# jyjblrd/Low-Cost-Mocap

Hardware: AMD Instinct MI355X
Metric: triangulated 3D markers/sec at 8 cams x 16 markers (higher is better)
Workload: dtype f64

## Files before the change

### low-cost-mocap_amd/csrc/frame_bb.hip

```cpp
#include "mocap_device.hpp"
#include "kernels.hpp"
#include <cstdlib>
#include "frame_common.hpp"
#include "bb_fold.hpp"

namespace mocap {

constexpr int kBBThreads = 256;
constexpr int kBBWaves = kBBThreads / 64;
constexpr int kBBRecs = kBBThreads + 64;
constexpr int bb_cw(int C) { return C <= 8 ? 1 : 2; }
constexpr uint32_t bb_rec_bytes(int CW) { return 24u + 8u * (uint32_t)CW; }
constexpr bool bb_group_rows(int CT, int ML, int RL) { return CT > 0 && ML > 0 && RL > 0 && CT * ML < 0xFF && (ML & (ML - 1)) == 0; }

constexpr int bb_wg_per_cu(int RL) { return RL == 48 ? 5 : 4; }
constexpr size_t kBBCacheEntry = 4;
constexpr int kBBLdsSlack = 1024;
struct BBLayout {
  size_t bxy, bxy_nx, cnt_nx, bt, rbound, seedkey, slot_key, claimw, recs, rpk, scr, scr_bytes, goff, gcnt, outslot, boff, bnb, seedgh, slot_g, cnt,
      misc, bpl, nh, hits, act, root_blob, root_cam, nact, bnl, bv, pkbase, seen, bcache, total;
  int ncache;
  __host__ __device__ static size_t al(size_t x, size_t a) { return (x + a - 1) / a * a; }
  __host__ __device__ BBLayout(int C, int M, int R, int CW, int wg_per_cu, bool row_words = false) {
    size_t o = 0;
    auto take = [&](size_t bytes, size_t a) {
      o = al(o, a);
      const size_t at = o;
      o += bytes;
      return at;
    };
    bxy = take(sizeof(float2) * (size_t)C * M, 16);
    bxy_nx = take(sizeof(float2) * (size_t)C * M, 16);
    cnt_nx = take(4 * (size_t)C, 4);
    bt = take(sizeof(double) * 10 * ((size_t)C * M + 1), 16);
    rbound = take(8 * (size_t)R, 8);
    claimw = take(8 * (size_t)C, 8);
    pkbase = take(8 * (size_t)CW * R, 8);
    scr = seedkey = take(8 * (size_t)R, 8);
    slot_key = take(8 * (size_t)kBBWaves * R, 8);
    recs = take(8 * (size_t)kBBRecs, 8);
    rpk = take(8 * (size_t)kBBRecs * CW, 8);
    seedgh = take(4 * (size_t)R, 4);
    slot_g = take(4 * (size_t)kBBWaves * R, 4);
    scr_bytes = o - scr;
    goff = take(4 * (size_t)(R + 1), 4);
    gcnt = take(4 * (size_t)R, 4);
    outslot = take(4 * (size_t)R, 4);
    boff = take(4 * (size_t)(R + 1), 4);
    bnb = take(4 * (size_t)R, 4);
    cnt = take(4 * (size_t)C, 4);
    misc = take(4 * 16, 4);
    bpl = take(2 * (size_t)R, 2);
    seen = take(2 * (size_t)R, 2);
    nh = take((size_t)R * C, row_words ? 8 : 1);
    hits = take((size_t)R * C * M, 1);
    act = take((size_t)R * C, row_words ? 8 : 1);
    root_blob = take((size_t)R, 1);
    root_cam = take((size_t)R, 1);
    nact = take((size_t)R, 1);
    bnl = take((size_t)R, 1);
    bv = take((size_t)R, 1);
    bcache = take(0, 4);
    ncache = 0;
    const size_t per_entry = kBBCacheEntry;
    for (int per_cu = wg_per_cu; per_cu >= 1; per_cu--) {
      const size_t lim = ((size_t)160 * 1024 / per_cu - kBBLdsSlack) / 256 * 256;
      if (lim >= o + per_entry * 64) {
        const size_t n = (lim - o) / per_entry;
        ncache = (int)(n > 1024 ? 1024 : n);
        break;
      }
    }
    o += per_entry * (size_t)ncache;
    total = al(o, 16);
  }
};

static int bb_fixed_slots(int C, int M, int R) {
  const char* e = getenv("MOCAP_BB_FIXED_LAYOUT");
  if (e && e[0] == '0') return 0;
  if (C == 8 && M == 16 && R <= 48) return 48;
  if (C == 8 && M == 16 && R <= 64) return 64;
  return 0;
}
static int frame_bb_root_slots(int C, int M, int R) {
  const int f = bb_fixed_slots(C, M, R);
  return f ? f : R;
}
size_t frame_bb_lds_bytes(int C, int M, int R) { return BBLayout(C, M, frame_bb_root_slots(C, M, R), bb_cw(C), bb_wg_per_cu(bb_fixed_slots(C, M, R)), bb_fixed_slots(C, M, R) != 0).total; }
static size_t frame_bb_lds_bytes_min(int C, int M, int R) {
  const BBLayout L(C, M, frame_bb_root_slots(C, M, R), bb_cw(C), bb_wg_per_cu(bb_fixed_slots(C, M, R)), bb_fixed_slots(C, M, R) != 0);
  return L.total - kBBCacheEntry * (size_t)L.ncache;
}
bool frame_bb_fits(int C, int M, int R) {
  return C >= 2 && C <= 16 && M >= 1 && M <= 64 && R >= 1 && R <= 255 && frame_bb_lds_bytes_min(C, M, R) <= (size_t)128 * 1024;
}

template <int CW, uint32_t NONE = 0xFFu>
struct Packed {
  unsigned long long w[CW];
  __device__ __forceinline__ void clear() {
#pragma unroll
    for (int k = 0; k < CW; k++) w[k] = NONE * 0x0101010101010101ull;
  }
  __device__ __forceinline__ void set(int c, uint32_t idx) {
    if (CW == 1)
      w[0] ^= (unsigned long long)(idx ^ NONE) << (8 * c);
    else
      w[c >> 3] ^= (unsigned long long)(idx ^ NONE) << (8 * (c & 7));
  }
  __device__ __forceinline__ uint32_t get(int c) const {
    return CW == 1 ? (uint32_t)(w[0] >> (8 * c)) & 0xFFu : (uint32_t)(w[c >> 3] >> (8 * (c & 7))) & 0xFFu;
  }
};

template <int CT, bool PERK = false>
struct BBCamTables {
  const double* base;
  static constexpr int C = CT;
  static constexpr int kPq = PERK ? 12 * CT * CT : 12 * CT;
  __device__ __forceinline__ ctab_t pq(size_t off) const { return as_ctab(base + off); }
  __device__ __forceinline__ ctab_t rt(size_t off) const { return as_ctab(base + kPq + off); }
  __device__ __forceinline__ ctab_t k4(size_t off) const { return as_ctab(base + kPq + 12 * CT + off); }
  __device__ __forceinline__ const double* f() const { return base + kPq + 16 * CT; }
};
template <bool PERK>
struct BBCamTables<0, PERK> {
  const double* base;
  int C;
  __device__ __forceinline__ ctab_t pq(size_t off) const { return as_ctab(base + off); }
  __device__ __forceinline__ ctab_t rt(size_t off) const { return as_ctab(base + (PERK ? 12 * C * C : 12 * C) + off); }
  __device__ __forceinline__ ctab_t k4(size_t off) const { return as_ctab(base + (PERK ? 12 * C * C + 12 * C : 24 * C) + off); }
  __device__ __forceinline__ const double* f() const { return base + (PERK ? 12 * C * C + 16 * C : 28 * C); }
};

enum { kPrioEval = 0, kPrioSeed = 1, kPrioPhase = 2, kPrioSerial = 3 };
template <int P>
__device__ __forceinline__ void bb_prio() {
  __builtin_amdgcn_s_setprio(P);
}

template <bool F32R, int CW, int CT, int ML, int RL, bool PERK = false>
struct BBState {
  static constexpr int T = kBBThreads, W = kBBWaves;
  static constexpr bool ROWS = bb_group_rows(CT, ML, RL);
  static constexpr uint32_t kNone = ROWS ? (uint32_t)(CT * ML) : 0xFFu;
  typedef Packed<CW, kNone> Pk;
  static_assert(!ROWS || (CT == 8 && CW == 1), "a row of nh / act as one word: eight cameras");
  __device__ __forceinline__ unsigned long long row_word64(const uint8_t* rows, int r) const { return ((const unsigned long long*)rows)[r]; }
  __device__ static __forceinline__ uint32_t byte_of(unsigned long long w, uint32_t k) { return (uint32_t)(w >> (8u * k)) & 0xFFu; }
  static constexpr bool PLIST = CT > 0 && ML > 0 && RL > 0 && ML < 32 && CT * ML <= 256 && (ML & (ML - 1)) == 0;
  __device__ __forceinline__ uint32_t gbyte(int c, uint32_t k) const { return ROWS ? (uint32_t)c * (uint32_t)ML + k : k; }
  __device__ __forceinline__ size_t grow(int c, uint32_t b) const { return ROWS ? (size_t)b : (size_t)c * M + b; }
  const FrameArgs& p;
  BBCamTables<CT, PERK> cv;
  const int C_, M, R, RS;
  int tid, lane, wave;
  __device__ __forceinline__ void fresh_tid() {
    int t = tid;
    asm volatile("" : "+v"(t));
    tid = t;
    lane = t & 63;
    wave = t >> 6;
  }
  __device__ __forceinline__ int cn() const { return CT > 0 ? CT : C_; }
  enum { PC_OTHER = 0, PC_PAIRS0, PC_PAIRS1, PC_B1_TABLE, PC_ROW_COPY, PC_PHASE_C, PC_SEED_PASS, PC_SEED_PUSH, PC_EVAL, PC_TEST, PC_PHASE_E, PC_COUNT };
#ifdef MOCAP_BB_PHASE_CLOCKS
  uint32_t pc_last = 0, pc_sum[PC_COUNT] = {};
  template <int PH>
  __device__ __forceinline__ void pc_mark() {
    if (__builtin_amdgcn_readfirstlane((int)threadIdx.x >> 6) == 0) {
      const uint32_t now = (uint32_t)__builtin_readcyclecounter();
      pc_sum[PH] += now - pc_last;
      pc_last = now;
    }
  }
  __device__ __forceinline__ void pc_start() { pc_last = (uint32_t)__builtin_readcyclecounter(); }
  __device__ __forceinline__ void pc_flush() const {
    if (threadIdx.x == 0 && !p.n_frames_dev)
      for (int k = 0; k < PC_COUNT; k++) atomicAdd(&p.status[p.n_frames + k], (int)(pc_sum[k] >> 8));
  }
#else
  template <int PH>
  __device__ __forceinline__ void pc_mark() {}
  __device__ __forceinline__ void pc_start() {}
  __device__ __forceinline__ void pc_flush() const {}
#endif
  double* bt;
  float2 *bxy, *bxy_nx;
  int32_t* cnt_nx;
  unsigned long long *rbound, *seedkey, *slot_key, *claimw, *rpk;
  struct BRec { uint32_t gh, rs; };
  BRec* recs;
  uint32_t *goff, *gcnt, *boff, *bnb, *seedgh, *slot_g;
  int32_t *outslot, *cnt, *misc;
  uint16_t* bpl;
  uint8_t *nh, *hits, *act, *root_blob, *root_cam, *nact, *bnl, *bv;
  float* bcache;
  unsigned long long* pkbase;
  uint16_t* seen;
  int ncache;
  unsigned char* scr;
  size_t scr_bytes;
  static constexpr unsigned long long kInfBits = 0x7ff0000000000000ull;

  __device__ BBState(const FrameArgs& p_, unsigned char* smem)
      : p(p_), C_(p_.cv.C), M(ML > 0 ? ML : p_.M), R(p_.K_max), RS(RL > 0 ? RL : p_.K_max), tid(threadIdx.x), lane(threadIdx.x & 63), wave(threadIdx.x >> 6) {
    const int C = cn();
    {
      const unsigned long long ta = (unsigned long long)(uintptr_t)p_.cv.Pq;
      uint32_t tlo = (uint32_t)__builtin_amdgcn_readfirstlane((int)(uint32_t)ta);
      uint32_t thi = (uint32_t)__builtin_amdgcn_readfirstlane((int)(uint32_t)(ta >> 32));
      asm volatile("" : "+s"(tlo), "+s"(thi));
      cv.base = (const double*)(uintptr_t)(((unsigned long long)thi << 32) | tlo);
      if constexpr (CT == 0) cv.C = C;
    }
    const BBLayout L(C, M, RS, CW, bb_wg_per_cu(RL), ROWS);
    bt = (double*)(smem + L.bt);
    bxy = (float2*)(smem + L.bxy);
    bxy_nx = (float2*)(smem + L.bxy_nx);
    cnt_nx = (int32_t*)(smem + L.cnt_nx);
    rbound = (unsigned long long*)(smem + L.rbound);
    seedkey = (unsigned long long*)(smem + L.seedkey);
    slot_key = (unsigned long long*)(smem + L.slot_key);
    claimw = (unsigned long long*)(smem + L.claimw);
    recs = (BRec*)(smem + L.recs);
    rpk = (unsigned long long*)(smem + L.rpk);
    goff = (uint32_t*)(smem + L.goff);
    gcnt = (uint32_t*)(smem + L.gcnt);
    outslot = (int32_t*)(smem + L.outslot);
    boff = (uint32_t*)(smem + L.boff);
    bnb = (uint32_t*)(smem + L.bnb);
    seedgh = (uint32_t*)(smem + L.seedgh);
    slot_g = (uint32_t*)(smem + L.slot_g);
    cnt = (int32_t*)(smem + L.cnt);
    misc = (int32_t*)(smem + L.misc);
    bpl = (uint16_t*)(smem + L.bpl);
    nh = (uint8_t*)(smem + L.nh);
    hits = (uint8_t*)(smem + L.hits);
    act = (uint8_t*)(smem + L.act);
    root_blob = (uint8_t*)(smem + L.root_blob);
    root_cam = (uint8_t*)(smem + L.root_cam);
    nact = (uint8_t*)(smem + L.nact);
    bnl = (uint8_t*)(smem + L.bnl);
    bv = (uint8_t*)(smem + L.bv);
    scr = smem + L.scr;
    scr_bytes = L.scr_bytes;
    bcache = (float*)(smem + L.bcache);
    pkbase = (unsigned long long*)(smem + L.pkbase);
    seen = (uint16_t*)(smem + L.seen);
    ncache = L.ncache;
  }

  struct Line { double a, b, c, den, rden; };
  __device__ __forceinline__ Line epiline(int r, int i) const { return epiline_of(root_cam[r], root_blob[r], i); }
  __device__ __forceinline__ Line epiline_of(int rc, int rb, int i) const {
    const int C = cn();
    const double* Fm = cv.f() + 9 * ((size_t)rc * C + i);
    const float2 rp = bxy[(size_t)rc * M + rb];
    const double x = (double)rp.x, y = (double)rp.y;
    double a = Fm[0] * x + Fm[1] * y + Fm[2];
    double b = Fm[3] * x + Fm[4] * y + Fm[5];
    double c = Fm[6] * x + Fm[7] * y + Fm[8];
    double nu = a * a + b * b;
    nu = nu != 0.0 ? 1.0 / sqrt(nu) : 1.0;
    a *= nu;
    b *= nu;
    c *= nu;
    if (F32R) {
      a = (double)(float)a;
      b = (double)(float)b;
      c = (double)(float)c;
    }
    Line L;
    L.a = a;
    L.b = b;
    L.c = c;
    L.den = sqrt(a * a + b * b);
    L.rden = recip_refined(L.den);
    return L;
  }

  template <bool CHAIN>
  __device__ __forceinline__ unsigned long long match_pairs(const Line& mine, int pair_r, int pair_i, int n_pairs, int gs_shift,
                                                            int cam = 0, int Mi_chain = 0) {
    const int C = cn();
    const int GS = 1 << gs_shift, PPS = 64 >> gs_shift;
    const int k = lane & (GS - 1), q = lane >> gs_shift;
    const int gl0 = lane & ~(GS - 1);
    const unsigned long long gall = gs_shift == 6 ? ~0ull : ((1ull << GS) - 1ull);
    unsigned long long claims = 0ull;
    for (int s0 = 0; s0 < n_pairs; s0 += PPS) {
      const int src = s0 + q;
      const bool has = src < n_pairs;
      const int sl = has ? src : 0;
      const double la = __shfl(mine.a, sl), lb = __shfl(mine.b, sl), lc = __shfl(mine.c, sl);
      const double lden = __shfl(mine.den, sl), lrden = __shfl(mine.rden, sl);
      const int r = __shfl(pair_r, sl);
      const int i = CHAIN ? cam : __shfl(pair_i, sl);
      const int Mi = has ? (CHAIN ? Mi_chain : cnt[i]) : 0;
      const bool valid = k < Mi;
      float2 pt = make_float2(0.f, 0.f);
      double d = 0.0;
      bool hit = false;
      if (valid) {
        pt = bxy[(size_t)i * M + k];
        const double num = fabs(la * (double)pt.x + lb * (double)pt.y + lc);
        d = div_by(num, lden, lrden);
        hit = d < p.gate_px;
      }
      const unsigned long long wm = __ballot(hit);
      const unsigned long long gm = (wm >> gl0) & gall;
      int rank = 0;
      const unsigned int dlo = (unsigned int)__double_as_longlong(d), dhi = (unsigned int)(__double_as_longlong(d) >> 32);
      for (unsigned long long mm = wm; mm;) {
        const int j = __ffsll((long long)mm) - 1;
        mm &= mm - 1;
        const double dj = __longlong_as_double(((long long)__builtin_amdgcn_readlane((int)dhi, j) << 32) |
                                               (unsigned int)__builtin_amdgcn_readlane((int)dlo, j));
        const bool mine_grp = (j & ~(GS - 1)) == gl0 && j != lane;
        rank += (hit && mine_grp && (dj < d || (dj == d && j < lane))) ? 1 : 0;
      }
      if (hit) hits[((size_t)r * C + i) * M + rank] = (uint8_t)gbyte(i, (uint32_t)k);
      const unsigned long long g0 = (__ballot(hit && rank == 0) >> gl0) & gall;
      bool same = false;
      if (valid && g0) {
        const float2 p0 = bxy[(size_t)i * M + (__ffsll((long long)g0) - 1)];
        same = pt.x == p0.x && pt.y == p0.y;
      }
      const unsigned long long cw = __ballot(same);
      if (CHAIN) {
        for (int sh = 0; sh < 64; sh += GS) claims |= (cw >> sh) & gall;
      }
      if (has && k == 0) {
        nh[(size_t)r * C + i] = (uint8_t)__popcll(gm);
        if (!CHAIN) {
          const unsigned long long cm = (cw >> gl0) & gall;
          if (cm) atomicOr(&claimw[i], cm);
        }
      }
    }
    return claims;
  }

  __device__ __forceinline__ void prefetch_lds(int64_t frame) const {
    const int C = cn();
    const float* src = p.blobs + (size_t)frame * C * M * 2;
    const int n_dw = C * M * 2;
    for (int base = wave * 64; base < n_dw; base += T)
      if (base + lane < n_dw)
        __builtin_amdgcn_global_load_lds((const __attribute__((address_space(1))) void*)(src + base + lane),
                                         (__attribute__((address_space(3))) void*)((float*)bxy_nx + base), 4, 0, 0);
    if (wave == 0 && lane < C)
      __builtin_amdgcn_global_load_lds((const __attribute__((address_space(1))) void*)(p.counts + (size_t)frame * C + lane),
                                       (__attribute__((address_space(3))) void*)cnt_nx, 4, 0, 0);
  }
  __device__ __forceinline__ void stage(int64_t frame) {
    fresh_tid();
    const int C = cn();
    float2* t = bxy;
    bxy = bxy_nx;
    bxy_nx = t;
    if (tid < C) {
      const int n = cnt_nx[tid];
      cnt[tid] = n < 0 ? 0 : (n > M ? M : n);
      claimw[tid] = 0ull;
    }
    if (tid == 0) {
      misc[MI_STATUS] = 0;
      misc[MI_OMAX] = 0;
    }
  }

  __device__ void match() {
    fresh_tid();
    const int C = cn();
    __syncthreads();
    int gs_shift = 0;
    while ((1 << gs_shift) < M) gs_shift++;
    const int n0 = cnt[0] < R ? cnt[0] : R;
    {
      for (int r = tid; r < n0; r += T) {
        root_cam[r] = 0;
        root_blob[r] = (uint8_t)r;
      }
      if (tid == 0 && cnt[0] > R) misc[MI_STATUS] |= MOCAP_ST_ROOT_OVERFLOW_;
    }
    __syncthreads();
    auto U_of = [&](int j) {
      const int n = cnt[j];
      return ~claimw[j] & (n >= 64 ? ~0ull : ((1ull << n) - 1ull));
    };
    int n_prov = 0, n_ppairs = 0;
    bool pre = false;
    uint8_t* nh_s = nullptr;
    uint8_t* hits_s = nullptr;
    unsigned long long* pclaim = (unsigned long long*)scr;
    uint8_t* plist = act;
    uint32_t* p_end = goff;
    {
      int Mmax = 0;
      for (int c = 1; c < C; c++) Mmax = cnt[c] > Mmax ? cnt[c] : Mmax;
#pragma nounroll
      for (int stage_ = 0; stage_ < 2; stage_++) {
        const int stage = __builtin_amdgcn_readfirstlane(stage_);
        int NP = n0 * (C - 1);
        if (stage == 1) {
          block_sync_lds();
          pc_mark<PC_PAIRS0>();
          if constexpr (PLIST) {
#pragma unroll
            for (int j = 1; j < CT; j++) {
              const uint32_t U = ~((const uint32_t*)claimw)[2 * j] & ((1u << cnt[j]) - 1u);
              if (lane < ML && ((U >> lane) & 1u)) plist[__builtin_amdgcn_mbcnt_lo(U, (uint32_t)n_prov)] = (uint8_t)(j * ML + lane);
              n_prov += __popc(U);
              n_ppairs += __popc(U) * (CT - 1 - j);
              if (lane == 0) p_end[j] = ((uint32_t)n_ppairs << 16) | (uint32_t)n_prov;
            }
            wave_lds_sync();
          } else
          for (int j = 1; j < C; j++) {
            const int np = __popcll(U_of(j));
            n_prov += np;
            n_ppairs += np * (C - 1 - j);
          }
          pre = n_prov <= 64 && (size_t)n_prov * C * (8 + 1 + (size_t)M) <= scr_bytes;
          if (!pre) break;
          nh_s = (uint8_t*)(pclaim + (size_t)n_prov * C);
          hits_s = nh_s + (size_t)n_prov * C;
          NP = n_ppairs;
        }
        for (int base = wave * 64; base < NP; base += W * 64) {
          const int pi = base + lane;
          const bool have = pi < NP;
          int r = 0, i = 1, Mi = 0;
          Line L = {0, 0, 0, 1, 1};
          if (have) {
            if (stage == 0) {
              r = pi / (C - 1);
              i = 1 + (pi - r * (C - 1));
              L = epiline(r, i);
            } else if constexpr (PLIST) {
              int j = 1;
              uint32_t before = 0;
              const uint32_t key = ((uint32_t)pi << 16) | 0xFFFFu;
              uint32_t pe[CT > 2 ? CT - 2 : 1];
#pragma unroll
              for (int jj = 1; jj <= CT - 2; jj++) pe[jj - 1] = p_end[jj];
#pragma unroll
              for (int jj = 1; jj <= CT - 2; jj++) {
                const bool ge = key >= pe[jj - 1];
                j += ge ? 1 : 0;
                before = ge ? pe[jj - 1] : before;
              }
              const uint32_t acc = before >> 16, pb = before & 0xFFFFu;
              uint32_t ord, off;
              divmod_tiny((uint32_t)pi - acc, (uint32_t)(CT - 1 - j), ord, off);
              r = (int)(pb + ord);
              const int k = plist[r] & (ML - 1);
              i = j + 1 + (int)off;
              L = epiline_of(j, k, i);
            } else {
              int j = 1, acc = 0, pb = 0, span = C - 2;
              unsigned long long U = 0ull;
              for (; j <= C - 2; j++) {
                span = C - 1 - j;
                U = U_of(j);
                const int nj = __popcll(U) * span;
                if (pi < acc + nj) break;
                acc += nj;
                pb += __popcll(U);
              }
              uint32_t ord, off;
              divmod_tiny((uint32_t)(pi - acc), (uint32_t)span, ord, off);
              for (uint32_t t = 0; t < ord; t++) U &= U - 1;
              const int k = __ffsll((long long)U) - 1;
              i = j + 1 + (int)off;
              r = pb + (int)ord;
              L = epiline_of(j, k, i);
            }
            Mi = cnt[i];
          }
          const float2* pts = bxy + (size_t)i * M;
          auto dist = [&](int k) {
            const float2 pt = pts[k];
            return div_by(fabs(L.a * (double)pt.x + L.b * (double)pt.y + L.c), L.den, L.rden);
          };
          unsigned long long hm = 0ull;
          double bd0 = __builtin_huge_val();
          int bk0 = 0;
          if constexpr (ROWS) {
#pragma unroll 4
            for (int k = 0; k < Mmax; k++)
              if (k < Mi) {
                const double d = dist(k);
                if (d < p.gate_px) {
                  hm |= 1ull << k;
                  if (d < bd0) {
                    bd0 = d;
                    bk0 = k;
                  }
                }
              }
          } else
#pragma unroll 4
          for (int k = 0; k < Mmax; k++)
            if (k < Mi && dist(k) < p.gate_px) hm |= 1ull << k;
          uint8_t* nhp = stage == 0 ? nh : nh_s;
          uint8_t* hl = (stage == 0 ? hits : hits_s) + ((size_t)r * C + i) * M;
          if (have) nhp[(size_t)r * C + i] = (uint8_t)__popcll(hm);
          unsigned long long rem = hm, claim = 0ull;
          int pos = 0;
          float2 p0 = make_float2(0.f, 0.f);
          if constexpr (ROWS) {
            if (hm) {
              hl[0] = (uint8_t)gbyte(i, (uint32_t)bk0);
              claim = hm;
              if (hm & (hm - 1ull)) {
                claim = 0ull;
                p0 = pts[bk0];
                for (unsigned long long t = hm; t; t &= t - 1) {
                  const int k = __ffsll((long long)t) - 1;
                  const float2 q = pts[k];
                  if (q.x == p0.x && q.y == p0.y) claim |= 1ull << k;
                }
              }
              rem = hm & ~(1ull << bk0);
              pos = 1;
            }
          }
          while (__ballot(rem != 0ull)) {
            if (rem) {
              double bd = __builtin_huge_val();
              int bk = 0;
              if (ROWS && !(rem & (rem - 1ull))) {
                bk = __ffsll((long long)rem) - 1;
              } else
              for (unsigned long long t = rem; t; t &= t - 1) {
                const int k = __ffsll((long long)t) - 1;
                const double d = dist(k);
                if (d < bd) {
                  bd = d;
                  bk = k;
                }
              }
              hl[pos] = (uint8_t)gbyte(i, (uint32_t)bk);
              if (!ROWS && pos == 0) {
                p0 = pts[bk];
                for (unsigned long long t = hm; t; t &= t - 1) {
                  const int k = __ffsll((long long)t) - 1;
                  const float2 q = pts[k];
                  if (q.x == p0.x && q.y == p0.y) claim |= 1ull << k;
                }
              }
              rem &= ~(1ull << bk);
              pos++;
            }
          }
          if (stage == 0) {
            if (claim) atomicOr(&claimw[i], claim);
          } else if (have) {
            pclaim[(size_t)r * C + i] = claim;
          }
        }
      }
    }
    const int NL = M * ((C - 1) * (C - 2) / 2);
    const bool spec = F32R && (size_t)NL * 20 + 8 <= scr_bytes;
    double* sp_den = (double*)scr;
    float* sp_abc = (float*)(sp_den + NL);
    auto sp_base = [&](int j) { return M * ((j - 1) * (C - 1) - (j - 1) * j / 2); };
    if (spec && !pre) {
      int tot = 0;
      for (int j = 1; j <= C - 2; j++) {
        const int n = cnt[j];
        const unsigned long long U = ~claimw[j] & (n >= 64 ? ~0ull : ((1ull << n) - 1ull));
        tot += __popcll(U) * (C - 1 - j);
      }
      for (int l = tid; l < tot; l += T) {
        int j = 1, acc = 0, span = C - 2;
        unsigned long long U = 0ull;
        for (; j <= C - 2; j++) {
          const int n = cnt[j];
          U = ~claimw[j] & (n >= 64 ? ~0ull : ((1ull << n) - 1ull));
          span = C - 1 - j;
          const int nj = __popcll(U) * span;
          if (l < acc + nj) break;
          acc += nj;
        }
        uint32_t ord, off;
        divmod_tiny((uint32_t)(l - acc), (uint32_t)span, ord, off);
        for (uint32_t t = 0; t < ord; t++) U &= U - 1;
        const int k = __ffsll((long long)U) - 1, i = j + 1 + (int)off;
        const int ll = sp_base(j) + k * span + (int)off;
        const Line L = epiline_of(j, k, i);
        sp_den[ll] = L.den;
        sp_abc[3 * ll + 0] = (float)L.a;
        sp_abc[3 * ll + 1] = (float)L.b;
        sp_abc[3 * ll + 2] = (float)L.c;
      }
    }
    __syncthreads();
    pc_mark<PC_PAIRS1>();
    fresh_tid();
    if (wave == 0) bb_prio<kPrioSerial>();
    if (wave == 0 && pre) {
      int jp = 0, kp = 0;
      if constexpr (PLIST) {
        if (lane < n_prov) {
          const int row = plist[lane];
          jp = row / ML;
          kp = row & (ML - 1);
        }
      } else
      if (lane < n_prov) {
        int acc = 0;
        unsigned long long U = 0ull;
        for (jp = 1; jp < C; jp++) {
          U = U_of(jp);
          const int np = __popcll(U);
          if (lane < acc + np) break;
          acc += np;
        }
        for (int t = 0; t < lane - acc; t++) U &= U - 1;
        kp = __ffsll((long long)U) - 1;
      }
      bool real = false;
      for (int i = 1; i < C; i++) {
        wave_lds_sync();
        if (lane < n_prov && jp == i) {
          real = !((claimw[i] >> kp) & 1ull);
          if (real)
            for (int c = i + 1; c < C; c++) {
              const unsigned long long m = pclaim[(size_t)lane * C + c];
              if (m) atomicOr(&claimw[c], m);
            }
        }
      }
      const unsigned long long rm = __ballot(real);
      const int rank = __popcll(rm & ((1ull << lane) - 1ull));
      int n_roots = n0 + __popcll(rm);
      if (real && n0 + rank < R) {
        root_cam[n0 + rank] = (uint8_t)jp;
        root_blob[n0 + rank] = (uint8_t)kp;
        bnl[rank] = (uint8_t)lane;
      }
      if (lane == 0) {
        if (n_roots > R) {
          misc[MI_STATUS] |= MOCAP_ST_ROOT_OVERFLOW_;
          n_roots = R;
        }
        misc[MI_NROOTS] = n_roots;
      }
    } else if (wave == 0) {
      const int cntL = lane < C ? cnt[lane] : 0;
      const unsigned long long clmL = lane < C ? claimw[lane] : 0ull;
      int nr_cam = 0, nr_blob = 0;
      int n_roots = n0;
      bool over = false;
      for (int i = 1; i < C; i++) {
        const int Mi = __builtin_amdgcn_readlane(cntL, i);
        unsigned long long claimed = ((unsigned long long)(unsigned int)__builtin_amdgcn_readlane((int)(clmL >> 32), i) << 32) |
                                     (unsigned int)__builtin_amdgcn_readlane((int)clmL, i);
        const int n_new = n_roots - n0;
        for (int base = 0; base < n_new; base += 64) {
          const int l = base + lane;
          const bool have = l < n_new;
          int j = nr_cam, k = nr_blob;
          if (base) {
            wave_lds_sync();
            j = have ? root_cam[n0 + l] : 0;
            k = have ? root_blob[n0 + l] : 0;
          }
          Line L = {0, 0, 0, 1, 1};
          if (have) {
            if (spec) {
              const int ll = sp_base(j) + k * (C - 1 - j) + (i - j - 1);
              L.a = (double)sp_abc[3 * ll + 0];
              L.b = (double)sp_abc[3 * ll + 1];
              L.c = (double)sp_abc[3 * ll + 2];
              L.den = sp_den[ll];
              L.rden = recip_refined(L.den);
            } else {
              L = epiline_of(j, k, i);
            }
          }
          claimed |= match_pairs<true>(L, n0 + l, i, (n_new - base < 64) ? n_new - base : 64, gs_shift, i, Mi);
        }
        const bool flag = lane < Mi && !((claimed >> lane) & 1ull);
        const unsigned long long mask = __ballot(flag);
        const int pos = __popcll(mask & ((1ull << lane) - 1ull));
        if (flag) {
          const int rr = n_roots + pos;
          if (rr < R) {
            root_cam[rr] = (uint8_t)i;
            root_blob[rr] = (uint8_t)lane;
          }
        }
        int slot = n_new;
        for (unsigned long long mm = mask; mm; slot++) {
          const int jb = __ffsll((long long)mm) - 1;
          mm &= mm - 1;
          if (lane == slot) {
            nr_cam = i;
            nr_blob = jb;
          }
        }
        n_roots += __popcll(mask);
        if (n_roots > R) {
          over = true;
          n_roots = R;
        }
      }
      if (lane == 0) {
        if (over) misc[MI_STATUS] |= MOCAP_ST_ROOT_OVERFLOW_;
        misc[MI_NROOTS] = n_roots;
      }
    } else {
      float om = 0.0f;
      for (int i = tid - 64; i < C * M; i += T - 64) {
        const int c = i / M, k = i - c * M;
        if (k < cnt[c]) {
          const float2 v = bxy[i];
          om = fmaxf(om, fmaxf(fabsf(v.x), fabsf(v.y)));
          double Bc[10];
          dlt_contribution(Bc, cv.pq(PERK ? 12 * (c * C + c) : 12 * c), (double)v.x, (double)v.y);
#pragma unroll
          for (int e = 0; e < 10; e++) bt[(size_t)i * 10 + e] = Bc[e];
        }
      }
      if (om > 0.0f) atomicMax(&misc[MI_OMAX], __float_as_int(om));
      if (tid == 64) {
        const int it = q_add(&p.q.counters[QC_NEXT_FRAME], 1);
        misc[MI_NEXT] = it < frame_count(p) ? it : -1;
      }
    }
    bb_prio<kPrioPhase>();
    __syncthreads();
    pc_mark<PC_B1_TABLE>();
    if (pre) {
      const int n_new = misc[MI_NROOTS] - n0;
      for (int idx = tid; idx < n_new * C; idx += T) {
        const int q = idx / C, c = idx - q * C;
        const int r = n0 + q, ps = bnl[q];
        if (c > (int)root_cam[r]) {
          const int n = nh_s[(size_t)ps * C + c];
          nh[(size_t)r * C + c] = (uint8_t)n;
          const uint8_t* src = hits_s + ((size_t)ps * C + c) * M;
          uint8_t* dst = hits + ((size_t)r * C + c) * M;
          for (int t = 0; t < n; t++) dst[t] = src[t];
        }
      }
      __syncthreads();
      pc_mark<PC_ROW_COPY>();
    }

    fresh_tid();
    const int nroots = misc[MI_NROOTS];
    for (int r = tid; r < nroots; r += T) {
      if constexpr (ROWS) {
        const uint32_t rc = root_cam[r], rb = root_blob[r];
        unsigned long long nw = row_word64(nh, r);
        const uint8_t* hr = hits + (size_t)r * (CT * ML);
        uint32_t h1[CT];
#pragma unroll
        for (int c = 1; c < CT; c++) h1[c] = hr[c * ML];
        nw &= (~0ull << (8u * rc)) << 8;
        Pk pkb;
        pkb.clear();
        pkb.set((int)rc, gbyte((int)rc, rb));
        static_assert(CT <= 8 && ML <= 16, "a digit's byte: three bits of camera, four of hit count - 1");
        unsigned long long ew = 0ull;
        uint32_t total = 1, views = 1, na = 0, sm = 1u << rc;
#pragma unroll
        for (int c = CT - 1; c >= 1; c--) {
          const uint32_t n = byte_of(nw, (uint32_t)c);
          if (n > 1) {
            ew = (ew << 8) | (unsigned long long)((n << 3) + (uint32_t)(c - 8));
            na++;
          }
          if (n == 1) pkb.set(c, h1[c]);
          if (n) {
            sm |= 1u << c;
            views++;
            total *= n;
          }
        }
        const unsigned long long aw = ew & 0x0707070707070707ull;
        const unsigned long long dn = ((ew >> 3) & 0x0F0F0F0F0F0F0F0Full) + 0x0101010101010101ull;
        const bool over = (unsigned long long)total > (unsigned long long)p.G_cap;
        if (over) atomicOr(&misc[MI_STATUS], MOCAP_ST_CAND_OVERFLOW_);
        ((unsigned long long*)act)[r] = aw;
        nact[r] = (uint8_t)na;
        bv[r] = (uint8_t)views;
        pkbase[r] = pkb.w[0];
        if (PERK) seen[r] = (uint16_t)sm;
        rbound[r] = kInfBits;
        const uint32_t g = (views > 1 && !over) ? total : 0u;
        gcnt[r] = g;
        uint32_t pl = 1, nb = over ? 1u : total;
        uint32_t nl = 0;
        while (nl < na && (pl < (uint32_t)p.bb_pl_min || (pl < (uint32_t)p.bb_pl && nb > (uint32_t)p.bb_nb_max))) {
          const uint32_t n = byte_of(dn, nl++);
          uint32_t dummy;
          pl *= n;
          divmod_small(nb, n, nb, dummy);
        }
        bpl[r] = (uint16_t)pl;
        bnl[r] = (uint8_t)nl;
        bnb[r] = g ? nb : 0u;
        seedkey[r] = 0ull;
        seedgh[r] = 0xFFFFFFFFu;
        continue;
      }
      const int rc = root_cam[r];
      unsigned long long total = 1;
      int views = 1, na = 0;
      bool over = false;
      Pk pkb;
      pkb.clear();
      pkb.set(rc, gbyte(rc, root_blob[r]));
      uint32_t sm = 1u << rc;
      for (int c = rc + 1; c < C; c++) {
        const unsigned n = nh[(size_t)r * C + c];
        if (n > 1) act[(size_t)r * C + na++] = (uint8_t)c;
        if (n == 1) pkb.set(c, hits[((size_t)r * C + c) * M]);
        if (n) {
          sm |= 1u << c;
          views++;
          total *= n;
          if (total > (unsigned long long)p.G_cap) {
            over = true;
            total = 1;
          }
        }
      }
      if (over) atomicOr(&misc[MI_STATUS], MOCAP_ST_CAND_OVERFLOW_);
      nact[r] = (uint8_t)na;
      bv[r] = (uint8_t)views;
#pragma unroll
      for (int k = 0; k < CW; k++) pkbase[(size_t)r * CW + k] = pkb.w[k];
      if (PERK) seen[r] = (uint16_t)sm;
      rbound[r] = kInfBits;
      const uint32_t g = (views > 1 && !over) ? (uint32_t)total : 0u;
      gcnt[r] = g;
      {
        const uint8_t* a = act + (size_t)r * C;
        uint32_t pl = 1, nb = 1;
        int nl = 0;
        for (int k = 0; k < na; k++) nb *= nh[(size_t)r * C + a[k]];
        if (over) nb = 1;
        while (nl < na && (pl < (uint32_t)p.bb_pl_min || (pl < (uint32_t)p.bb_pl && nb > (uint32_t)p.bb_nb_max))) {
          const uint32_t n = nh[(size_t)r * C + a[nl++]];
          uint32_t dummy;
          pl *= n;
          divmod_small(nb, n, nb, dummy);
        }
        bpl[r] = (uint16_t)pl;
        bnl[r] = (uint8_t)nl;
        bnb[r] = g ? nb : 0u;
        seedkey[r] = 0ull;
        seedgh[r] = 0xFFFFFFFFu;
      }
    }
    for (int s = tid; s < W * RS; s += T) {
      slot_key[s] = ~0ull;
      slot_g[s] = 0xFFFFFFFFu;
    }
    if (tid == 0) misc[MI_BBCTR] = misc[MI_BBCTR2] = 0;
    __syncthreads();
    if (wave == 0) bb_prio<kPrioSerial>();
    if (wave == 0) {
      uint32_t carry = 0, bcarry = 0;
      int slots = 0;
      for (int base = 0; base < nroots; base += 64) {
        const int r = base + lane;
        const uint32_t g = r < nroots ? gcnt[r] : 0u;
        const uint32_t nb = r < nroots ? bnb[r] : 0u;
        const uint32_t incl = wave_inclusive_scan(g, lane);
        const uint32_t bincl = wave_inclusive_scan(nb, lane);
        const unsigned long long nz = __ballot(g != 0u);
        if (r < nroots) {
          goff[r] = carry + incl - g;
          boff[r] = bcarry + bincl - nb;
          outslot[r] = g ? slots + __popcll(nz & ((1ull << lane) - 1ull)) : -1;
        }
        carry += (uint32_t)__builtin_amdgcn_readlane((int)incl, 63);
        bcarry += (uint32_t)__builtin_amdgcn_readlane((int)bincl, 63);
        slots += __popcll(nz);
      }
      if (lane == 0) {
        goff[nroots] = carry;
        boff[nroots] = bcarry;
        misc[MI_NOUT] = slots;
        misc[MI_G] = misc[MI_STATUS] ? 0 : (int32_t)carry;
      }
    }
    bb_prio<kPrioPhase>();
    __syncthreads();
    pc_mark<PC_PHASE_C>();
  }

  __device__ __forceinline__ void add_view(double (&B)[10], int c, uint32_t k, int j) const {
    if (PERK && j != c) {
      const float2 w = bxy[grow(c, k)];
      double Bc[10];
      dlt_contribution(Bc, cv.base + 12 * ((size_t)j * cn() + c), (double)w.x, (double)w.y);
#pragma unroll
      for (int e = 0; e < 10; e++) B[e] = B[e] + Bc[e];
    } else {
      const double* t = bt + grow(c, k) * 10;
#pragma unroll
      for (int e = 0; e < 10; e++) B[e] = B[e] + t[e];
    }
  }

  template <bool WITH_B>
  __device__ __forceinline__ int group_matrix(int r, uint32_t rem, int skip, double (&B)[10], Pk& pk) const {
    const int C = cn();
    const int rc = root_cam[r];
    const uint8_t* nhr = nh + (size_t)r * C;
    const uint8_t* hr = hits + (size_t)r * C * M;
    pk.clear();
    int v = 0, ka = 0;
    int j = 0;
    if (WITH_B) {
#pragma unroll
      for (int e = 0; e < 10; e++) B[e] = 0.0;
    }
    for (int c = 0; c < C; c++) {
      uint32_t k = kNone;
      bool seen = false;
      if (c == rc) {
        k = gbyte(c, root_blob[r]);
        seen = true;
      } else if (c > rc) {
        const uint32_t n = nhr[c];
        seen = n != 0;
        if (n == 1) {
          k = hr[(size_t)c * M];
        } else if (n > 1) {
          if (ka >= skip) {
            uint32_t qd, dgt;
            if (rem < 8192u) divmod_tiny(rem, n, qd, dgt); else
            divmod_small(rem, n, qd, dgt);
            rem = qd;
            k = hr[(size_t)c * M + dgt];
          }
          ka++;
        }
      }
      if (k != kNone) {
        if (WITH_B) add_view(B, c, k, j);
        v++;
        pk.set(c, k);
      }
      if (PERK) j += seen ? 1 : 0;
    }
    return v;
  }

  __device__ __forceinline__ void block_pk(int r, uint32_t gh, Pk& pk) const {
    const int C = cn();
#pragma unroll
    for (int k = 0; k < CW; k++) pk.w[k] = pkbase[(size_t)r * CW + k];
    if constexpr (ROWS) {
      const unsigned long long aw = row_word64(act, r), nw = row_word64(nh, r);
      const int na = nact[r];
      const uint8_t* hr = hits + (size_t)r * (CT * ML);
      uint32_t rem = gh;
      for (int k = bnl[r]; k < na; k++) {
        const uint32_t c = byte_of(aw, (uint32_t)k), n = byte_of(nw, c);
        uint32_t qd, dgt;
        if (rem < 8192u) divmod_tiny(rem, n, qd, dgt); else
        divmod_small(rem, n, qd, dgt);
        rem = qd;
        pk.set((int)c, hr[c * (uint32_t)ML + dgt]);
      }
      return;
    }
    const uint8_t* a = act + (size_t)r * C;
    const int na = nact[r];
    uint32_t rem = gh;
    for (int k = bnl[r]; k < na; k++) {
      const int c = a[k];
      const uint32_t n = nh[(size_t)r * C + c];
      uint32_t qd, dgt;
      if (rem < 8192u) divmod_tiny(rem, n, qd, dgt); else
      divmod_small(rem, n, qd, dgt);
      rem = qd;
      pk.set(c, hits[((size_t)r * C + c) * M + dgt]);
    }
  }
  __device__ __forceinline__ int block_matrix(int r, uint32_t gh, Pk& pk, double (&B)[10]) const {
    const int C = cn();
    block_pk(r, gh, pk);
#pragma unroll
    for (int ee = 0; ee < 10; ee++) B[ee] = 0.0;
    if constexpr (PERK) {
      const uint32_t sm = seen[r];
#pragma unroll CT > 0 ? CT : 1
      for (int c = 0; c < C; c++) {
        const uint32_t k = pk.get(c);
        if (k != kNone) add_view(B, c, k, __popc(sm & ((1u << c) - 1u)));
      }
    } else {
#pragma unroll CT > 0 ? CT : 1
      for (int c = 0; c < C; c++) {
        const uint32_t k = pk.get(c);
        const double* t = bt + (size_t)(ROWS ? k : k != 0xFFu ? (uint32_t)c * (uint32_t)M + k : (uint32_t)C * (uint32_t)M) * 10;
#pragma unroll
        for (int ee = 0; ee < 10; ee++) B[ee] = B[ee] + t[ee];
      }
    }
    return (int)bv[r] - (int)bnl[r];
  }

  __device__ __forceinline__ int fetch_candidate(uint32_t lo, uint32_t i, int& r, uint32_t& gl, Pk& pk, double (&B)[10]) const {
    const int C = cn();
    const BRec rec = recs[lo];
    r = (int)(rec.rs & 0xFFu);
#pragma unroll
    for (int k = 0; k < CW; k++) pk.w[k] = rpk[(size_t)lo * CW + k];
    if (rec.rs >> 31) {
      gl = rec.gh;
    } else {
      uint32_t rem = i - (rec.rs >> 8);
      gl = rec.gh * (uint32_t)bpl[r] + rem;
      const uint8_t* a = act + (size_t)r * C;
      const int nl = bnl[r];
      if constexpr (ROWS) {
        const unsigned long long aw = row_word64(act, r), nw = row_word64(nh, r);
        const uint8_t* hr = hits + (size_t)r * (CT * ML);
        for (int k = 0; k < nl; k++) {
          const uint32_t c = byte_of(aw, (uint32_t)k);
          uint32_t qd, dgt;
          divmod_tiny(rem, byte_of(nw, c), qd, dgt);
          rem = qd;
          pk.set((int)c, hr[c * (uint32_t)ML + dgt]);
        }
      } else
      for (int k = 0; k < nl; k++) {
        const int c = a[k];
        uint32_t qd, dgt;
        divmod_tiny(rem, nh[(size_t)r * C + c], qd, dgt);
        rem = qd;
        pk.set(c, hits[((size_t)r * C + c) * M + dgt]);
      }
    }
#pragma unroll
    for (int ee = 0; ee < 10; ee++) B[ee] = 0.0;
    if constexpr (PERK) {
      int j = 0;
#pragma unroll CT > 0 ? CT : 1
      for (int c = 0; c < C; c++) {
        const uint32_t k = pk.get(c);
        if (k != kNone) add_view(B, c, k, j++);
      }
    } else {
#pragma unroll CT > 0 ? CT : 1
      for (int c = 0; c < C; c++) {
        const uint32_t k = pk.get(c);
        const double* t = bt + (size_t)(ROWS ? k : k != 0xFFu ? (uint32_t)c * (uint32_t)M + k : (uint32_t)C * (uint32_t)M) * 10;
#pragma unroll
        for (int ee = 0; ee < 10; ee++) B[ee] = B[ee] + t[ee];
      }
    }
    return bv[r];
  }

  __device__ void search(bool bound_tests) {
    fresh_tid();
    const int C = cn();
    (void)C;
    __builtin_amdgcn_s_waitcnt(0x0F70);
    const int nroots = misc[MI_NROOTS];
    int32_t* ctr = &misc[MI_BBCTR];
    int32_t* ctr_other = &misc[MI_BBCTR2];
    const double inf = __builtin_huge_val();
    EigCut ec;
    {
      const double om = (double)__int_as_float(misc[MI_OMAX]);
      ec.p3max2 = p.p3max2;
      ec.o2slack = (1100.0 * 0x1p-46) * (om * om);
    }
    const double c0[3] = {p.bb_c0[0], p.bb_c0[1], p.bb_c0[2]};
    const uint32_t nblocks = boff[nroots];
    auto root_of_block = [&](uint32_t b_first_of_wave, uint32_t b) {
      return coop_last_le([&](int r) { return boff[r]; }, nroots, b_first_of_wave, b, lane);
    };
    auto push_block = [&](int r, uint32_t gh, const Pk& pk) {
      const uint32_t old = (uint32_t)atomicAdd(ctr, (int32_t)(((uint32_t)bpl[r] << 10) | 1u));
      const uint32_t slot = old & 0x3FFu;
      BRec rec;
      rec.gh = gh;
      rec.rs = (uint32_t)r | ((old >> 10) << 8);
      recs[slot] = rec;
#pragma unroll
      for (int k = 0; k < CW; k++) rpk[(size_t)slot * CW + k] = pk.w[k];
    };
    auto rec_start = [&](int k) { return (recs[k].rs & 0x7FFFFFFFu) >> 8; };
    auto root_y = [&](int r) {
      const int vf = bv[r];
      const double bound = __longlong_as_double((long long)rbound[r]);
      const double limit = bound * (double)(2 * vf) * (1.0 + 0x1p-40);
      const double limit_adj = fma(1.002, limit, (double)(2 * vf) * ec.o2slack);
      return p.p3max2c * limit_adj;
    };
    auto dropped = [&](int r, double s1, double tr) { return s1 * fma(2e-12, tr, root_y(r)) < 1.0; };
    if (bound_tests) {
      bb_prio<kPrioSeed>();
      int my_r = -1;
      uint32_t my_gh = 0;
      unsigned long long my_key = 0ull;
      Pk my_pk;
      my_pk.clear();
      for (uint32_t s0 = 0; s0 < nblocks; s0 += T) {
        const uint32_t b = s0 + (uint32_t)tid;
        if (s0 + (uint32_t)(wave * 64) >= nblocks) continue;
        const int r = root_of_block(s0 + (uint32_t)(wave * 64), b < nblocks ? b : nblocks - 1);
        if (b < nblocks) {
          const uint32_t gh = b - boff[r];
          double B[10], tr = 0.0;
          Pk pk;
          const int v = block_matrix(r, gh, pk, B);
          double s1d = __builtin_huge_val();
          float s1 = 0.0f;
          if (v >= 2) {
            s1d = eigcut_s1_shifted(B, c0, tr);
            s1 = (float)fmin(s1d, 3e38);
          }
          if (b < (uint32_t)ncache) bcache[b] = v >= 2 ? bb_fold_bound(s1d, tr) : bb_fold_inf();
          my_key = ((unsigned long long)__float_as_uint(s1) << 32) | (unsigned long long)(0xFFFFFFFFu - gh);
          my_r = r;
          my_gh = gh;
          my_pk = pk;
          atomicMax(&seedkey[r], my_key);
        }
      }
      block_sync_lds_only();
      pc_mark<PC_SEED_PASS>();
      if (nblocks <= (uint32_t)T) {
        if (my_r >= 0 && seedkey[my_r] == my_key) {
          seedgh[my_r] = my_gh;
          push_block(my_r, my_gh, my_pk);
        }
      } else
      for (int r = tid; r < nroots; r += T) {
        if (bnb[r]) {
          const uint32_t gh = 0xFFFFFFFFu - (uint32_t)seedkey[r];
          seedgh[r] = gh;
          seedkey[r] = 0ull;
          Pk pk;
          block_pk(r, gh, pk);
          push_block(r, gh, pk);
        }
      }
      bb_prio<kPrioEval>();
      block_sync_lds_only();
      pc_mark<PC_SEED_PUSH>();
    }
    uint32_t b0 = 0;
    fresh_tid();
    while (true) {
      const uint32_t cv_ = (uint32_t)*ctr;
      const uint32_t ns = cv_ & 0x3FFu, ne = cv_ >> 10;
      const bool blocks_left = b0 < nblocks;
      const bool full = ns > (uint32_t)(kBBRecs - T);
      if (ns && (full || !blocks_left || ne >= (uint32_t)p.bb_flush)) {
        for (uint32_t i0 = 0; i0 < ne; i0 += T) {
          const uint32_t i = i0 + (uint32_t)tid;
          const bool have = i < ne;
          double e = inf, X[3] = {0, 0, 0};
          int r = 0;
          uint32_t gl = 0;
          uint32_t lo = 0;
          if (i0 + (uint32_t)(wave * 64) < ne)
            lo = (uint32_t)coop_last_le(rec_start, (int)ns, i0 + (uint32_t)(wave * 64), have ? i : ne - 1, lane);
          Pk pk;
          pk.clear();
          if (have) {
            double B[10];
            const int v = fetch_candidate(lo, i, r, gl, pk, B);
            if constexpr (ROWS) {
#pragma unroll
              for (int k = 0; k < CW; k++) asm volatile("" : "+v"(pk.w[k]));
            }
            auto obs_p = [&](int c, double& x, double& y) -> bool {
              const uint32_t k = pk.get(c);
              if (k == kNone) return false;
              const float2 w = bxy[grow(c, k)];
              x = (double)w.x;
              y = (double)w.y;
              return true;
            };
            const double bound = __longlong_as_double((long long)rbound[r]);
            solve_and_score<!PERK, true, F32R, false, 1, true>(cv, B, v, obs_p, X, e, bound * (double)(2 * v) * (1.0 + 0x1p-40), ec);
#ifdef MOCAP_DEBUG_EIGCHECK
            if (!(e < inf)) {
              double B2[10], X2[3], e2;
#pragma unroll
              for (int ee = 0; ee < 10; ee++) B2[ee] = 0.0;
              int j2 = 0;
              for (int c = 0; c < C; c++) {
                const uint32_t k = pk.get(c);
                if (k != kNone) add_view(B2, c, k, j2++);
              }
              solve_and_score<!PERK, true, F32R>(cv, B2, v, obs_p, X2, e2);
              atomicAdd(&p.status[p.n_frames], 1);
              if (e2 <= bound) printf("EIGCHECK candidate: root %d g %u bound %.17g true %.17g\n", r, gl, bound, e2);
            }
#endif
          }
          const bool fin = e < inf;
          const unsigned long long key = fin ? (unsigned long long)__double_as_longlong(e) : kInfBits;
          const uint32_t gword = (gl << 1) | ((e != e) ? 1u : 0u);
          const int ss = wave * RS + r;
          if (fin) atomicMin(&rbound[r], key);
          const bool want = have && (key < slot_key[ss] || (key == slot_key[ss] && gword < slot_g[ss]));
          if (__ballot(want)) {
            unsigned long long old = 0;
            if (want) old = atomicMin(&slot_key[ss], key);
            wave_lds_sync();
            const bool holder = want && slot_key[ss] == key;
            if (holder && old > key) slot_g[ss] = 0xFFFFFFFFu;
            wave_lds_sync();
            if (holder) atomicMin(&slot_g[ss], gword);
            wave_lds_sync();
            if (holder && slot_g[ss] == gword) store_winner(ss, X, pk);
          }
        }
        block_sync_lds_only();
        pc_mark<PC_EVAL>();
        if (tid == 0) *ctr = 0;
        {
          int32_t* t = ctr;
          ctr = ctr_other;
          ctr_other = t;
        }
        continue;
      }
      if (!blocks_left) break;
      const uint32_t b = b0 + (uint32_t)tid;
      const uint32_t bw = b0 + (uint32_t)(wave * 64);
      b0 += T;
      int r = 0;
      if (bw < nblocks) r = root_of_block(bw, b < nblocks ? b : nblocks - 1);
      bool do_push = false;
      uint32_t gh = 0;
      Pk pk;
      pk.clear();
      if (b < nblocks) {
        gh = b - boff[r];
        if (gh != seedgh[r]) {
          double B[10], tr;
          bool survive = true;
          if (bound_tests && b < (uint32_t)ncache) {
            survive = !bb_fold_dropped(bcache[b], root_y(r));
            if (survive) block_pk(r, gh, pk);
          } else if (bound_tests) {
            const int v = block_matrix(r, gh, pk, B);
            if (v >= 2) {
              const double s1 = eigcut_s1_shifted(B, c0, tr);
              survive = !dropped(r, s1, tr);
            }
          } else {
            block_pk(r, gh, pk);
          }
          do_push = survive;
#ifdef MOCAP_DEBUG_EIGCHECK
          if (!survive) {
            const double bound = __longlong_as_double((long long)rbound[r]);
            const uint32_t pl = bpl[r];
            for (uint32_t l = 0; l < pl; l++) {
              double B2[10], X2[3], e2 = inf;
              Pk pk2;
              const int v2 = group_matrix<true>(r, gh * pl + l, 0, B2, pk2);
              auto obs2 = [&](int c, double& x, double& y) -> bool {
                const uint32_t k = pk2.get(c);
                if (k == kNone) return false;
                const float2 w = bxy[grow(c, k)];
                x = (double)w.x;
                y = (double)w.y;
                return true;
              };
              solve_and_score<!PERK, true, F32R>(cv, B2, v2, obs2, X2, e2);
              atomicAdd(&p.status[p.n_frames + 1], 1);
              if (e2 <= bound) printf("EIGCHECK block: root %d block %u candidate %u bound %.17g true %.17g\n", r, gh, l, bound, e2);
            }
          }
#endif
        }
      }
      block_sync_lds_only();
      if (do_push) push_block(r, gh, pk);
      block_sync_lds_only();
      pc_mark<PC_TEST>();
    }
    wait_own_stores();
    __syncthreads();
  }

  __device__ __forceinline__ bool root_winner(int r, unsigned long long& kb, uint32_t& gw, int& wb) const {
    kb = ~0ull;
    gw = 0xFFFFFFFFu;
    wb = 0;
    for (int w = 0; w < W; w++) {
      const int s = w * RS + r;
      const unsigned long long k = slot_key[s];
      const uint32_t g = slot_g[s];
      if (k < kb || (k == kb && g < gw)) {
        kb = k;
        gw = g;
        wb = w;
      }
    }
    return kb != ~0ull;
  }

  static constexpr uint32_t kRecBytes = bb_rec_bytes(CW);
  __device__ __forceinline__ unsigned char* winner_rec(int s) const {
    return p.ws + (size_t)blockIdx.x * p.ws_stride + (size_t)(kRecBytes * (uint32_t)s);
  }
  __device__ __forceinline__ void store_winner(int s, const double (&X)[3], const Pk& pk) const {
    unsigned long long* rec = (unsigned long long*)winner_rec(s);
    if constexpr (CW == 1) {
      typedef unsigned long long rec2_t __attribute__((ext_vector_type(2)));
      const rec2_t lo = {(unsigned long long)__double_as_longlong(X[0]), (unsigned long long)__double_as_longlong(X[1])};
      const rec2_t hi = {(unsigned long long)__double_as_longlong(X[2]), pk.w[0]};
      ((rec2_t*)rec)[0] = lo;
      ((rec2_t*)rec)[1] = hi;
    } else {
#pragma unroll
      for (int k = 0; k < 3; k++) rec[k] = (unsigned long long)__double_as_longlong(X[k]);
#pragma unroll
      for (int k = 0; k < CW; k++) rec[3 + k] = pk.w[k];
    }
  }
  __device__ static __forceinline__ uint32_t row_word(uint32_t two) {
    const uint32_t x = (two & 0xFFu) | ((two & 0xFF00u) << 8);
    if constexpr (ROWS) {
      static_assert(!ROWS || kNone == 0x80u, "row_word: the record of zeros is the byte with bit 7 set");
      return (x & ((uint32_t)(ML - 1) * 0x00010001u)) | ((x >> 7) & 0x00010001u) * 0xFFFFu;
    }
    const uint32_t none = ((x + 0x00010001u) >> 8) & 0x00010001u;
    return x | none * 0xFF00u;
  }
  __device__ void write_point(int64_t frame, int r) const {
    const int C = cn();
    unsigned long long kb;
    uint32_t gw;
    int wv;
    if (!root_winner(r, kb, gw, wv)) return;
    const double e = kb != kInfBits ? __longlong_as_double((long long)kb)
                                    : ((gw & 1u) ? __longlong_as_double(0x7ff8000000000000ll) : __builtin_huge_val());
    const size_t o = (size_t)frame * R + outslot[r];
    const unsigned long long* rec = (const unsigned long long*)winner_rec(wv * RS + r);
    unsigned long long w[3 + CW];
#pragma unroll
    for (int k = 0; k < 3 + CW; k++) w[k] = q_ld(rec + k);
    p.err[o] = e;
    const double X[3] = {__longlong_as_double((long long)w[0]), __longlong_as_double((long long)w[1]), __longlong_as_double((long long)w[2])};
    int16_t* co = p.corr + o * C;
    if constexpr (CT == 8) {
      typedef uint32_t row_t __attribute__((ext_vector_type(4), aligned(2)));
      const uint32_t lo = (uint32_t)w[3], hi = (uint32_t)(w[3] >> 32);
      row_t v = {row_word(lo), row_word(lo >> 16), row_word(hi), row_word(hi >> 16)};
      *(row_t*)co = v;
    } else {
      for (int c = 0; c < C; c++) {
        const uint32_t k = (uint32_t)(w[3 + (CW == 1 ? 0 : c >> 3)] >> (8 * (c & 7))) & 0xFFu;
        co[c] = k == kNone ? (int16_t)-1 : (int16_t)(ROWS ? k & (uint32_t)(ML - 1) : k);
      }
    }
    store_point(p, o, X);
  }
};

template <bool F32R, int CW, int CT, int ML, int RL>
__global__ __launch_bounds__(kBBThreads, bb_wg_per_cu(RL)) void frame_bb_kernel(FrameArgs p) {
  extern __shared__ __attribute__((aligned(16))) unsigned char smem[];
#define BB_STATE BBState<F32R, CW, CT, ML, RL>
#include "frame_bb_body.inc"
#undef BB_STATE
}

template <bool F32R, int CW, int CT, int ML, int RL>
__global__ __launch_bounds__(kBBThreads, bb_wg_per_cu(RL)) void frame_bb_calib_kernel(FrameArgs p) {
  extern __shared__ __attribute__((aligned(16))) unsigned char smem[];
#define BB_STATE BBState<F32R, CW, CT, ML, RL, true>
#include "frame_bb_body.inc"
#undef BB_STATE
}

int frame_bb_wg_per_cu_cap(int C, int M, int R) { return bb_wg_per_cu(bb_fixed_slots(C, M, R)); }
size_t frame_bb_ws_bytes(int) { return BBLayout::al(bb_rec_bytes(2) * (size_t)kBBWaves * 255, 256); }
static_assert(bb_wg_per_cu(48) <= kBBMaxWgPerCu && bb_wg_per_cu(64) <= kBBMaxWgPerCu && bb_wg_per_cu(0) <= kBBMaxWgPerCu, "frame_capi.hip sizes the workspace for kBBMaxWgPerCu workgroups per CU");

hipError_t launch_frame_bb(const FrameArgs& a, int grid, hipStream_t stream) {
  const size_t lds = frame_bb_lds_bytes(a.cv.C, a.M, a.K_max);
  if (!a.ws || a.ws_stride < bb_rec_bytes(bb_cw(a.cv.C)) * (size_t)kBBWaves * (size_t)frame_bb_root_slots(a.cv.C, a.M, a.K_max)) return hipErrorInvalidValue;
  const size_t nPq = a.cv.uniformK ? (size_t)12 * a.cv.C : (size_t)12 * a.cv.C * a.cv.C;
  if (a.cv.RT != a.cv.Pq + nPq || a.cv.K4 != a.cv.RT + 12 * a.cv.C || a.cv.F != a.cv.K4 + 4 * a.cv.C) return hipErrorInvalidValue;
  void (*k)(FrameArgs);
  const bool f32 = a.cv.f32_rounding != 0;
  const int fixed = bb_fixed_slots(a.cv.C, a.M, a.K_max);
  if (fixed && fixed != 48 && fixed != 64) return hipErrorInvalidValue;
  static_assert(bb_cw(8) == 1 && bb_cw(9) == 2 && bb_cw(16) == 2, "BB_PICK takes CW = 1 up to eight cameras, CW = 2 above");
#define BB_PICK(KERNEL)                                                                             \
  (fixed == 48       ? (f32 ? KERNEL<true, 1, 8, 16, 48> : KERNEL<false, 1, 8, 16, 48>)             \
   : fixed == 64     ? (f32 ? KERNEL<true, 1, 8, 16, 64> : KERNEL<false, 1, 8, 16, 64>)             \
   : a.cv.C == 8     ? (f32 ? KERNEL<true, 1, 8, 0, 0> : KERNEL<false, 1, 8, 0, 0>)                 \
   : a.cv.C <= 8     ? (f32 ? KERNEL<true, 1, 0, 0, 0> : KERNEL<false, 1, 0, 0, 0>)                 \
                     : (f32 ? KERNEL<true, 2, 0, 0, 0> : KERNEL<false, 2, 0, 0, 0>))
  k = a.cv.uniformK ? BB_PICK(frame_bb_kernel) : BB_PICK(frame_bb_calib_kernel);
#undef BB_PICK
  if (lds > 48 * 1024) {
    hipError_t e = hipFuncSetAttribute((const void*)k, hipFuncAttributeMaxDynamicSharedMemorySize, (int)lds);
    if (e != hipSuccess) return e;
  }
  hipLaunchKernelGGL(k, dim3(grid), dim3(kBBThreads), lds, stream, a);
  return hipGetLastError();
}

}
```

Baseline: 649.6 million.

## Prefilter epipolar gating with conservative f32 bound, then exact f64 check on candidates

In the ROWS path, blob distances to the epiline are first screened in f32 against a threshold that is rounded up and widened by an error bound. The bound uses a wave-wide max of point magnitudes computed with DPP reductions. Only candidate blobs that pass the screen are re-evaluated with the exact f64 distance, and the loop iterates while any lane still has candidates. The non-F32R path instead loads two blobs per float4 and updates the running best without branches. This aims to cut the f64 arithmetic and divergent branching in the hot gating loop, at the cost of extra reduction work per call and reliance on the error bound being conservative.

```diff
diff --git a/low-cost-mocap_amd/csrc/frame_bb.hip b/low-cost-mocap_amd/csrc/frame_bb.hip
--- a/low-cost-mocap_amd/csrc/frame_bb.hip
+++ b/low-cost-mocap_amd/csrc/frame_bb.hip
@@ -140,6 +140,12 @@
   __builtin_amdgcn_s_setprio(P);
 }
 
+__device__ __forceinline__ float f32_round_up(double v) {
+  const float f = (float)v;
+  const int32_t b = __float_as_int(f);
+  return (double)f < v ? __int_as_float(b + ((b >> 31) | 1)) : f;
+}
+
 template <bool F32R, int CW, int CT, int ML, int RL, bool PERK = false>
 struct BBState {
   static constexpr int T = kBBThreads, W = kBBWaves;
@@ -490,18 +496,75 @@
           double bd0 = __builtin_huge_val();
           int bk0 = 0;
           if constexpr (ROWS) {
-#pragma unroll 4
-            for (int k = 0; k < Mmax; k++)
-              if (k < Mi) {
-                const double d = dist(k);
-                if (d < p.gate_px) {
-                  hm |= 1ull << k;
-                  if (d < bd0) {
-                    bd0 = d;
-                    bk0 = k;
+            static_assert(ML % 2 == 0 && ML < 32, "two blobs per word, the slots as bits of one register");
+            const float4* pw = (const float4*)pts;
+            uint32_t cand = (1u << Mi) - 1u;
+            uint32_t hw = 0u;
+            if constexpr (F32R) {
+              static_assert(CT * ML == 128, "the frame's slots: one word of two blobs per lane");
+              uint32_t ob;
+              {
+                const float4 v = ((const float4*)bxy)[lane];
+                const int n = cnt[lane / (ML / 2)], k0 = 2 * (lane % (ML / 2));
+                const uint32_t ax = __float_as_uint(v.x) & 0x7FFFFFFFu, ay = __float_as_uint(v.y) & 0x7FFFFFFFu;
+                const uint32_t az = __float_as_uint(v.z) & 0x7FFFFFFFu, aw = __float_as_uint(v.w) & 0x7FFFFFFFu;
+                const uint32_t m0 = k0 < n ? (ax > ay ? ax : ay) : 0u, m1 = k0 + 1 < n ? (az > aw ? az : aw) : 0u;
+                ob = m0 > m1 ? m0 : m1;
+                auto up = [](uint32_t x, uint32_t y) { return x > y ? x : y; };
+                ob = up(ob, (uint32_t)__builtin_amdgcn_update_dpp(0, (int)ob, 0xB1, 0xf, 0xf, true));
+                ob = up(ob, (uint32_t)__builtin_amdgcn_update_dpp(0, (int)ob, 0x4E, 0xf, 0xf, true));
+                ob = up(ob, (uint32_t)__builtin_amdgcn_update_dpp(0, (int)ob, 0x141, 0xf, 0xf, true));
+                ob = up(ob, (uint32_t)__builtin_amdgcn_update_dpp(0, (int)ob, 0x140, 0xf, 0xf, true));
+                const uint32_t r0 = (uint32_t)__builtin_amdgcn_readlane((int)ob, 0), r1 = (uint32_t)__builtin_amdgcn_readlane((int)ob, 16);
+                const uint32_t r2 = (uint32_t)__builtin_amdgcn_readlane((int)ob, 32), r3 = (uint32_t)__builtin_amdgcn_readlane((int)ob, 48);
+                ob = up(up(r0, r1), up(r2, r3));
+                ob = ob < 0x7F800000u ? ob : 0x7F800000u;
+              }
+              const double om = (double)__uint_as_float(ob);
+              const float a32 = (float)L.a, b32 = (float)L.b, c32 = (float)L.c;
+              const float thr = f32_round_up(p.gate_px * L.den * (1.0 + 1e-12) + (2.5 * 0x1p-24) * (2.0 * om + fabs(L.c)) * (1.0 + 1e-6));
+              uint32_t pm = 0u;
+#pragma unroll
+              for (int h = ML / 2 - 1; h >= 0; h--) {
+                const float4 v = pw[h];
+                float t0 = fmaf(a32, v.x, fmaf(b32, v.y, c32)), t1 = fmaf(a32, v.z, fmaf(b32, v.w, c32));
+                asm("" : "+v"(t0), "+v"(t1));
+                pm = pm + pm + (fabsf(t1) <= thr ? 1u : 0u);
+                pm = pm + pm + (fabsf(t0) <= thr ? 1u : 0u);
+              }
+              cand &= pm;
+              while (__ballot(cand != 0u)) {
+                if (cand) {
+                  const int k = __ffs((int)cand) - 1;
+                  cand &= cand - 1u;
+                  const double d = dist(k);
+                  if (d < p.gate_px) {
+                    hw |= 1u << k;
+                    if (d < bd0) {
+                      bd0 = d;
+                      bk0 = k;
+                    }
                   }
                 }
               }
+            } else {
+#pragma unroll
+              for (int h = 0; h < ML / 2; h++) {
+                const float4 v = pw[h];
+                const double d0 = div_by(fabs(L.a * (double)v.x + L.b * (double)v.y + L.c), L.den, L.rden);
+                const double d1 = div_by(fabs(L.a * (double)v.z + L.b * (double)v.w + L.c), L.den, L.rden);
+                const bool h0 = d0 < p.gate_px && ((cand >> (2 * h)) & 1u), h1 = d1 < p.gate_px && ((cand >> (2 * h + 1)) & 1u);
+                hw |= h0 ? 1u << (2 * h) : 0u;
+                const bool b0 = h0 && d0 < bd0;
+                bd0 = b0 ? d0 : bd0;
+                bk0 = b0 ? 2 * h : bk0;
+                hw |= h1 ? 2u << (2 * h) : 0u;
+                const bool b1 = h1 && d1 < bd0;
+                bd0 = b1 ? d1 : bd0;
+                bk0 = b1 ? 2 * h + 1 : bk0;
+              }
+            }
+            hm = hw;
           } else
 #pragma unroll 4
           for (int k = 0; k < Mmax; k++)
```

Measured after the change: 667.3 million, median of 6. 1.03x the previous value.
